# rlog58/dags-vae-search

Hardware: AMD Instinct MI355X
Metric: DAGs/sec VAE+predictor train step, n=12 batch 4096 per GPU, at 1 MI355X (higher is better)
Workload: dtype f32 (fwd bf16x6, bwd bf16x3 split products, fp32 accumulate); 1 GPU; synthetic_v12 DAGs (n=12, card=12, N=15 tokens), PACE-VAE train step: pack + fwd + bwd + clip_grad_norm_(1.0) + Adam(1e-4), train mode dropout 0.15; per_gpu_batch=4096, global_batch=4096, waves_per_workgroup=8, parallelism=single

## Files before the change

### dags_vae_search_amd/csrc/dvs_stage.h

```cpp
#pragma once
#include "dvs_device.h"

constexpr int DVS_PLAN_VECS = 6;
struct DvsStagePlan {
    const f4* src;
    int dst16;
    int n16;
    const float* vsrc[DVS_PLAN_VECS];
    unsigned short vdst[DVS_PLAN_VECS];
    unsigned short vbase[DVS_PLAN_VECS];
    unsigned short vlen[DVS_PLAN_VECS];
    int vperm;
    int nvec;
    int zero_int;
    int phase;
    const float* cold[2];
    int cold_tiles;
};

#ifdef DVS_STAMPS
constexpr int DVS_STAMP_IDS = 8, DVS_STAMP_PHASES = 32, DVS_STAMP_WAVES = 8, DVS_STAMP_WGS = 256;
#define DVS_STAMP_DECL(name) __device__ unsigned long long name[DVS_STAMP_WGS * DVS_STAMP_WAVES * DVS_STAMP_PHASES * DVS_STAMP_IDS]
#define DVS_STAMP(buf, pp, id)                                                                                              \
    do {                                                                                                                    \
        if ((dvs_tid() & 63) == 0 && dvs_bid() < DVS_STAMP_WGS && (dvs_tid() >> 6) < DVS_STAMP_WAVES)                        \
            buf[(((size_t)dvs_bid() * DVS_STAMP_WAVES + (dvs_tid() >> 6)) * DVS_STAMP_PHASES + ((pp)->phase & 31)) *          \
                    DVS_STAMP_IDS + (id)] = __builtin_amdgcn_s_memtime();                                                    \
    } while (0)
#define DVS_ACC_STAMP_DECL(name) __device__ unsigned long long name[256 * 8 * 8]
#define DVS_ACC_STAMP_AT(buf, last, nw, ids, k)                                                                             \
    do {                                                                                                                    \
        const unsigned long long now_ = __builtin_amdgcn_s_memtime();                                                       \
        if ((dvs_tid() & 63) == 0 && dvs_bid() < 256) buf[(dvs_bid() * (nw) + (dvs_tid() >> 6)) * (ids) + (k)] += now_ - last; \
        last = now_;                                                                                                        \
    } while (0)
#define DVS_ACC_STAMP(buf, last, k) DVS_ACC_STAMP_AT(buf, last, 8, 8, k)
#define DVS_STAMP_READER(name)                                                                                              \
    extern "C" int dvs_debug_read_stamps_##name(void* out, size_t bytes, int clear) {                                       \
        if (bytes > sizeof(dvs_stamps_##name)) bytes = sizeof(dvs_stamps_##name);                                           \
        if (hipMemcpyFromSymbol(out, HIP_SYMBOL(dvs_stamps_##name), bytes) != hipSuccess) return 1;                         \
        void* p = nullptr;                                                                                                  \
        if (clear && (hipGetSymbolAddress(&p, HIP_SYMBOL(dvs_stamps_##name)) != hipSuccess ||                               \
                      hipMemset(p, 0, sizeof(dvs_stamps_##name)) != hipSuccess))                                            \
            return 2;                                                                                                       \
        return 0;                                                                                                           \
    }
#else
#define DVS_STAMP(buf, pp, id) ((void)0)
#define DVS_ACC_STAMP(buf, last, k) ((void)0)
#define DVS_ACC_STAMP_AT(buf, last, nw, ids, k) ((void)0)
#endif

#ifndef DVS_EMU
#define DVS_HD __host__ __device__
#else
#define DVS_HD
#endif
#define DVS_FAKE_LDS ((char*)(uintptr_t)(1u << 20))
DVS_HD inline void dvs_plan_clear(DvsStagePlan& p) {
    p.src = nullptr;
    p.dst16 = 0;
    p.n16 = 0;
    for (int i = 0; i < DVS_PLAN_VECS; ++i) {
        p.vsrc[i] = nullptr;
        p.vdst[i] = 0;
        p.vbase[i] = 0;
        p.vlen[i] = 0;
    }
    p.phase = 0;
    p.nvec = 0;
    p.vperm = 0;
    p.zero_int = -1;
    p.cold[0] = p.cold[1] = nullptr;
    p.cold_tiles = 0;
}
DVS_HD inline void dvs_plan_cold(DvsStagePlan& p, const float* a, const float* b, int tiles) {
    p.cold[0] = a ? a : b;
    p.cold[1] = b ? b : a;
    p.cold_tiles = (a || b) ? tiles : 0;
}
DVS_HD inline void dvs_plan_seg(DvsStagePlan& p, const char* smem, const void* lds_dst, const void* src, int n_bf16) {
    p.src = (const f4*)src;
    p.dst16 = (int)(((const char*)lds_dst - smem) >> 4);
    p.n16 = n_bf16 >> 3;
}
DVS_HD inline void dvs_plan_vec(DvsStagePlan& p, const char* smem, const float* lds_dst, const float* src, int n,
                                bool perm = false) {
    for (int base = 0; base < n; base += 64) {
        if (p.nvec >= DVS_PLAN_VECS) {
            p.nvec = DVS_PLAN_VECS + 1;
            return;
        }
        p.vsrc[p.nvec] = src;
        p.vdst[p.nvec] = (unsigned short)(((const char*)lds_dst - smem) >> 2);
        p.vbase[p.nvec] = (unsigned short)base;
        p.vlen[p.nvec] = (unsigned short)n;
        if (perm) p.vperm |= 1 << p.nvec;
        ++p.nvec;
    }
}

constexpr int DVS_PF_THREADS = 256;
constexpr int DVS_PF_BWD = 9, DVS_PF_FWD = 14, DVS_PF_BWD_TAIL = 18, DVS_PF_FWD_TAIL = 27;
template <int NCH>
struct DvsPrefetch {
    f4 v[NCH];
    float s[2];
};

#ifndef DVS_EMU
typedef const __attribute__((address_space(4))) DvsStagePlan* DvsPlanK;
#else
typedef const DvsStagePlan* DvsPlanK;
#endif

DVS_HD inline bool dvs_plan_ok(const DvsStagePlan& p) { return p.nvec <= DVS_PLAN_VECS; }
void dvs_note_hip_error(const char* what, int hip_error, const char* hip_message);
DVS_HD inline void dvs_plan_seal(DvsStagePlan& p) {
#if !defined(__HIP_DEVICE_COMPILE__)
    if (!dvs_plan_ok(p)) {
        dvs_note_hip_error("staging plan", -1, "more than DVS_PLAN_VECS vector units (launcher bug)");
        p.nvec = DVS_PLAN_VECS;
    }
#endif
    for (int i = 0; i < DVS_PLAN_VECS; ++i)
        if (i >= p.nvec || !p.vsrc[i] || p.vlen[i] <= 0) {
            p.vsrc[i] = (const float*)p.src;
            p.vbase[i] = 0;
            p.vlen[i] = 0;
        }
}

__device__ __forceinline__ int dvs_uniform(int v) {
#ifndef DVS_EMU
    return __builtin_amdgcn_readfirstlane(v);
#else
    return v;
#endif
}
struct DvsPlanHead {
    const char* src;
    int dst, nwc, rot, wave, nw, lane16;
};
template <bool ROT, class PP>
__device__ __forceinline__ DvsPlanHead dvs_plan_head(PP p, int tid, int step) {
    DvsPlanHead h;
    h.src = (const char*)p->src;
    h.dst = p->dst16 * 16;
    h.nwc = p->n16 >> 6;
    h.rot = ROT ? (int)(((unsigned)dvs_bid() * 2654435761u) % (unsigned)(h.nwc > 0 ? h.nwc : 1)) : 0;
    h.wave = dvs_uniform(tid >> 6);
    h.nw = step >> 6;
    h.lane16 = (tid & 63) * 16;
    return h;
}
template <bool ROT>
__device__ __forceinline__ bool dvs_plan_slot(const DvsPlanHead& h, int u, int& byte) {
    int c = u * h.nw + h.wave;
    const bool live = c < h.nwc;
    if (ROT) {
        c += h.rot;
        c = c >= h.nwc ? c - h.nwc : c;
    }
    byte = ((live ? c : 0) << 10) + h.lane16;
    return live;
}

template <bool ROT, int NCH, class PP>
__device__ __forceinline__ void dvs_prefetch_issue(DvsPrefetch<NCH>& pf, PP p, int tid, int step) {
    const DvsPlanHead h = dvs_plan_head<ROT>(p, tid, step);
#pragma unroll
    for (int u = 0; u < NCH; ++u) {
        int byte;
        dvs_plan_slot<ROT>(h, u, byte);
        pf.v[u] = *(const f4*)(h.src + (unsigned)byte);
    }
#pragma unroll
    for (int q = 0; q < 2; ++q) {
        const int j = h.wave + q * h.nw, jc = j < DVS_PLAN_VECS ? j : 0;
        const int idx = p->vbase[jc] + (tid & 63);
        const int ic = (j < DVS_PLAN_VECS && idx < p->vlen[jc]) ? idx : 0;
        pf.s[q] = p->vsrc[jc][((p->vperm >> jc) & 1) ? dvs_pi(ic) : ic];
    }
}
template <bool ROT, int NCH, class PP>
__device__ __forceinline__ void dvs_prefetch_commit(const DvsPrefetch<NCH>& pf, PP p, char* smem, int tid, int step) {
    const DvsPlanHead h = dvs_plan_head<ROT>(p, tid, step);
#pragma unroll
    for (int u = 0; u < NCH; ++u) {
        int byte;
        if (dvs_plan_slot<ROT>(h, u, byte)) *(f4*)(smem + h.dst + byte) = pf.v[u];
    }
    float* ldsf = (float*)smem;
#pragma unroll
    for (int q = 0; q < 2; ++q) {
        const int j = h.wave + q * h.nw, jc = j < DVS_PLAN_VECS ? j : 0;
        const int idx = p->vbase[jc] + (tid & 63);
        if (j < DVS_PLAN_VECS && idx < p->vlen[jc]) ldsf[p->vdst[jc] + idx] = pf.s[q];
    }
    if (p->zero_int >= 0 && tid < 2) ((int*)smem)[p->zero_int + tid] = 0;
}
struct DvsTouch {
    float v[2];
};
template <class PP>
__device__ __forceinline__ DvsTouch dvs_touch_first(PP next, bool has_next, int nw, int wave, int lane) {
    DvsTouch t;
    t.v[0] = t.v[1] = 0.f;
    if (has_next && next->cold_tiles > 0) {
        int tile = dvs_bid() * nw + wave;
        tile = tile < next->cold_tiles ? tile : 0;
        const size_t off = (size_t)tile * 1024 + (size_t)lane * 16;
        t.v[0] = next->cold[0][off];
        t.v[1] = next->cold[1][off];
    }
    return t;
}
__device__ __forceinline__ void dvs_touch_done(const DvsTouch& t) {
#ifndef DVS_EMU
    asm volatile("" ::"v"(t.v[0]), "v"(t.v[1]));
#else
    (void)t;
#endif
}

template <int NCH, class PP>
__device__ __forceinline__ void dvs_stage_now(PP p, char* smem) {
    DvsPrefetch<NCH> pf;
    dvs_prefetch_issue<true>(pf, p, dvs_tid(), (int)blockDim.x);
    dvs_prefetch_commit<true>(pf, p, smem, dvs_tid(), (int)blockDim.x);
}
```

### dags_vae_search_amd/csrc/k_forward.hip

```cpp
#include "dvs_kernels.h"
#include "dvs_wimg.h"

constexpr int PACK_DAGS = 4;
__device__ __forceinline__ void pack_stream(float* dst, const float* __restrict__ src, size_t nfloats) {
    const size_t n4 = nfloats >> 2;
    size_t i = threadIdx.x;
    for (; i + 3 * blockDim.x < n4; i += 4 * blockDim.x) {
        f4 v[4];
#pragma unroll
        for (int u = 0; u < 4; ++u) v[u] = *(const f4*)(src + 4 * (i + u * blockDim.x));
#pragma unroll
        for (int u = 0; u < 4; ++u) *(f4*)(dst + 4 * (i + u * blockDim.x)) = v[u];
    }
    for (; i < n4; i += blockDim.x) *(f4*)(dst + 4 * i) = *(const f4*)(src + 4 * i);
    for (size_t i = 4 * n4 + threadIdx.x; i < nfloats; i += blockDim.x) dst[i] = src[i];
}
__global__ __launch_bounds__(8 * 16 * PACK_DAGS) void k_pack(PackArgs a) {
    DVS_DYN_LDS(smem);
    const int N = a.N, C = a.C;
    const int dag0 = blockIdx.x * PACK_DAGS;
    const int nd = (a.B - dag0 < PACK_DAGS) ? a.B - dag0 : PACK_DAGS;
    float* s_lab = (float*)smem;
    float* s_pos = s_lab + PACK_DAGS * 16 * 16;
    float* s_adj = s_pos + PACK_DAGS * 16 * 16;
    float* s_msk = s_adj + PACK_DAGS * 16 * 16;
    {
        const float* src[4] = {a.lab1h + (size_t)dag0 * N * C, a.pos1h + (size_t)dag0 * N * N, a.adj + (size_t)dag0 * N * N,
                               (const float*)(a.tmask + (size_t)dag0 * 8 * N * N)};
        float* dst[4] = {s_lab, s_pos, s_adj, s_msk};
        const int nf[4] = {nd * N * C, nd * N * N, nd * N * N, nd * 8 * N * N / 4};
        bool whole = true;
#pragma unroll
        for (int k = 0; k < 4; ++k) whole = whole && (nf[k] & 3) == 0 && (nf[k] >> 2) <= 2 * (int)blockDim.x;
        if (whole) {
            f4 v[4][2];
#pragma unroll
            for (int k = 0; k < 4; ++k)
#pragma unroll
                for (int u = 0; u < 2; ++u) {
                    const int i = (int)threadIdx.x + u * (int)blockDim.x;
                    v[k][u] = *(const f4*)(src[k] + 4 * (i < (nf[k] >> 2) ? i : 0));
                }
#pragma unroll
            for (int k = 0; k < 4; ++k)
#pragma unroll
                for (int u = 0; u < 2; ++u) {
                    const int i = (int)threadIdx.x + u * (int)blockDim.x;
                    if (i < (nf[k] >> 2)) *(f4*)(dst[k] + 4 * i) = v[k][u];
                }
        } else {
#pragma unroll
            for (int k = 0; k < 4; ++k) pack_stream(dst[k], src[k], (size_t)nf[k]);
        }
    }
    __syncthreads();
    const int h = threadIdx.x / (16 * PACK_DAGS), d = (threadIdx.x >> 4) % PACK_DAGS, i = threadIdx.x & 15;
    if (d >= nd) return;
    const uint8_t* msk = (const uint8_t*)s_msk;
    int bad = 0;
    if (h > 0) {
        if (i < N) {
            const uint8_t* m0 = msk + ((size_t)d * 8 * N + i) * N;
            const uint8_t* mh = msk + (((size_t)d * 8 + h) * N + i) * N;
            for (int j = 0; j < N; ++j)
                if ((mh[j] != 0) != (m0[j] != 0)) bad |= 2;
        }
        if (bad) atomicOr(a.status, bad);
        return;
    }
    int label = 0, pos = 0;
    unsigned parents = 0, allowed = 1u << i;
    if (i < N) {
        const float* lr = s_lab + ((size_t)d * N + i) * C;
        int ones = 0;
        for (int c = 0; c < C; ++c) {
            const float v = lr[c];
            if (v == 1.0f) { label = c; ++ones; } else if (v != 0.0f) bad |= 1;
        }
        if (ones != 1) bad |= 1;
        const float* pr = s_pos + ((size_t)d * N + i) * N;
        ones = 0;
        for (int c = 0; c < N; ++c) {
            const float v = pr[c];
            if (v == 1.0f) { pos = c; ++ones; } else if (v != 0.0f) bad |= 1;
        }
        if (ones != 1) bad |= 1;
        const float* ad = s_adj + (size_t)d * N * N;
        for (int j = 0; j < N; ++j)
            if (ad[j * N + i] != 0.0f) parents |= 1u << j;
        allowed = 0;
        const uint8_t* m0 = msk + ((size_t)d * 8 * N + i) * N;
        for (int j = 0; j < N; ++j)
            if (!m0[j]) allowed |= 1u << j;
        if (!((allowed >> i) & 1u)) bad |= 4;
    }
    DvsRecord* r = a.rec + dag0 + d;
    r->label[i] = (uint8_t)label;
    r->pos[i] = (uint8_t)pos;
    r->parents[i] = (uint16_t)parents;
    r->allowed[i] = (uint16_t)allowed;
    if (bad) atomicOr(a.status, bad);
}

void dvs_launch_pack(const PackArgs& a, dvs_stream_t st) {
    const size_t lds = (size_t)PACK_DAGS * (3 * 256 * 4 + 8 * 256);
    DVS_SET_LDS(k_pack, lds);
    DVS_LAUNCH(k_pack, dim3((a.B + PACK_DAGS - 1) / PACK_DAGS), dim3(8 * 16 * PACK_DAGS), lds, st, a);
}

__global__ __launch_bounds__(256) void k_build_records(BuildArgs a) {
    __shared__ unsigned short s_child[16][256];
    __shared__ unsigned short s_reach[16][256];
    __shared__ unsigned char s_indeg[16][256];
    __shared__ unsigned char s_order[16][256];
    const int tid = threadIdx.x;
    const int dag = blockIdx.x * 256 + tid;
    if (dag >= a.B) return;
    const int N = a.N, n = N - 3, out_id = N - 1;
    int bad = 0;
    for (int v = 0; v < 16; ++v) s_child[v][tid] = 0;
    s_child[0][tid] = 1u << 1;
    unsigned haspred = 0;
    for (int v = 0; v < n; ++v) {
        const unsigned p = a.preds[(size_t)dag * n + v];
        if (p >> v) bad |= 8;
        for (int u = 0; u < v; ++u)
            if ((p >> u) & 1u) s_child[u + 2][tid] |= (unsigned short)(1u << (v + 2));
        if (p & ((1u << v) - 1u)) haspred |= 1u << v;
    }
    for (int v = 0; v < n; ++v)
        if (!((haspred >> v) & 1u)) s_child[1][tid] |= (unsigned short)(1u << (v + 2));
    for (int v = 0; v < N - 1; ++v)
        if (s_child[v][tid] == 0) s_child[v][tid] = (unsigned short)(1u << out_id);
    for (int v = 0; v < 16; ++v) s_indeg[v][tid] = 0;
    for (int u = 0; u < N; ++u) {
        unsigned c = s_child[u][tid];
        while (c) {
            const int v = __ffs((int)c) - 1;
            c &= c - 1;
            s_indeg[v][tid]++;
        }
    }
    int tail = 0;
    for (int v = 0; v < N; ++v)
        if (s_indeg[v][tid] == 0) s_order[tail++][tid] = (unsigned char)v;
    for (int head = 0; head < tail && head < N; ++head) {
        unsigned c = s_child[s_order[head][tid]][tid];
        while (c) {
            const int v = __ffs((int)c) - 1;
            c &= c - 1;
            if (--s_indeg[v][tid] == 0 && tail < 16) s_order[tail++][tid] = (unsigned char)v;
        }
    }
    if (tail != N) bad |= 8;
    for (int v = 0; v < N; ++v) s_reach[v][tid] = (unsigned short)(s_child[v][tid] | (1u << v));
    for (int k = 0; k < N; ++k) {
        const unsigned rk = s_reach[k][tid];
        for (int v = 0; v < N; ++v)
            if ((s_reach[v][tid] >> k) & 1u) s_reach[v][tid] |= (unsigned short)rk;
    }
    DvsRecord* r = a.rec + dag;
    for (int i = 0; i < 16; ++i) {
        int label = 0, pos = 0;
        unsigned parents = 0, allowed = 1u << i;
        if (i < N) {
            if (i == 0) label = 2;
            else if (i == 1) label = 0;
            else if (i == out_id) label = 1;
            else {
                label = a.labels[(size_t)dag * n + (i - 2)] + 3;
                if (label >= a.C) { bad |= 1; label = 0; }
            }
            pos = s_order[i][tid];
            allowed = 0;
            for (int j = 0; j < N; ++j) {
                if ((s_child[j][tid] >> i) & 1u) parents |= 1u << j;
                if ((s_reach[j][tid] >> i) & 1u) allowed |= 1u << j;
            }
        }
        r->label[i] = (uint8_t)label;
        r->pos[i] = (uint8_t)pos;
        r->parents[i] = (uint16_t)parents;
        r->allowed[i] = (uint16_t)allowed;
    }
    if (bad) atomicOr(a.status, bad);
}

void dvs_launch_build_records(const BuildArgs& a, dvs_stream_t st) {
    DVS_LAUNCH(k_build_records, dim3((a.B + 255) / 256), dim3(256), 0, st, a);
}

struct EmbLds {
    float *W1, *W2, *labw, *labb, *scr;
};
__device__ __forceinline__ EmbLds emb_lds(char* smem) {
    EmbLds l;
    l.W1 = (float*)smem;
    l.W2 = l.W1 + 2 * DVS_MAXTOK * DVS_LD;
    l.labw = l.W2 + 64 * EMB_LDW2;
    l.labb = l.labw + 32 * 16;
    l.scr = l.labb + 32;
    return l;
}
static size_t emb_lds_floats(int nwaves) {
    const size_t n = 2 * DVS_MAXTOK * DVS_LD + 64 * EMB_LDW2 + 32 * 16 + 32 + (size_t)nwaves * 16;
    return n > (size_t)DvsEmbImg::FLOATS ? n : (size_t)DvsEmbImg::FLOATS;
}

__global__ __launch_bounds__(1024) void k_embed_fwd(EmbedArgs a, DvsStagePlan plan) {
    DVS_DYN_LDS(smem);
    const int N = a.dims.N, C = a.dims.C;
    const EmbLds l = emb_lds(smem);
    if (blockDim.x >= 1024) dvs_stage_now<2>(&plan, smem);
    else dvs_stage_now<5>(&plan, smem);
    __syncthreads();
    const Lane L = dvs_lane();
    const DvsDrop D = dvs_drop_of(a.dims);
    float* scr = l.scr + L.wave * 16;
    for (int dag = blockIdx.x * L.nwaves + L.wave; dag < a.dims.B; dag += gridDim.x * L.nwaves) {
        const DvsRecord* rec = a.rec + dag;
        const bool valid = L.r < N;
        const EmbSel sel = dvs_emb_selectors(rec, N, scr, L);
        f4 eh[4];
        dvs_emb_hidden(eh, l.W1, N, sel, L);
        const uint32_t gdag = a.dims.dag_offset + dag;
        const int label = rec->label[L.r];
        for (int v = 0; v < (a.out2 ? 2 : 1); ++v) {
            const int site = v ? a.site2 : a.site;
            f4 e1[4];
#pragma unroll
            for (int t = 0; t < 4; ++t) e1[t] = eh[t];
            dvs_dropout_tile(e1, dvs_site_key(a.dims.seed_lo, a.dims.seed_hi, site, gdag), D, L);
            f4 x[4];
            f4 e2[2] = {f4_zero(), f4_zero()};
#pragma unroll
            for (int t = 0; t < 4; ++t) {
                const f4 w0 = dvs_wcol(l.W2, EMB_LDW2, 0, t, L), w1 = dvs_wcol(l.W2, EMB_LDW2, 16, t, L);
#pragma unroll
                for (int kk = 0; kk < 4; ++kk) {
                    e2[0] = dvs_mfma(w0[kk], e1[t][kk], e2[0]);
                    e2[1] = dvs_mfma(w1[kk], e1[t][kk], e2[1]);
                }
            }
            {
                f4 tmp[2] = {e2[0], e2[1]};
                dvs_dropout_tile<2>(tmp, dvs_site_key(a.dims.seed_lo, a.dims.seed_hi, site + 1, gdag), D, L);
                x[2] = tmp[0];
                x[3] = tmp[1];
            }
#pragma unroll
            for (int t = 0; t < 2; ++t)
#pragma unroll
                for (int kk = 0; kk < 4; ++kk) {
                    const int f = 16 * t + 4 * L.g + kk;
                    x[t][kk] = valid ? fmaxf(l.labw[f * 16 + label] + l.labb[f], 0.f) : 0.f;
                }
            if (!valid) { x[2] = f4_zero(); x[3] = f4_zero(); }
            dvs_store_tile(v ? a.out2 : a.out, dag, x, L);
        }
    }
}

void dvs_launch_embed_fwd(const EmbedArgs& a, int grid, int nw, dvs_stream_t st) {
    const size_t lds = emb_lds_floats(16) * 4;
    DvsStagePlan plan;
    dvs_plan_clear(plan);
    dvs_plan_seg(plan, DVS_FAKE_LDS, DVS_FAKE_LDS, a.embimg, 2 * DvsEmbImg::FLOATS);
    dvs_plan_seal(plan);
    DVS_SET_LDS(k_embed_fwd, lds);
    DVS_LAUNCH(k_embed_fwd, dim3(grid), dim3(nw == 4 ? 256 : 1024), lds, st, a, plan);
}

#ifdef DVS_STAMPS
DVS_STAMP_DECL(dvs_stamps_fwd);
struct DvsLatTag { int phase; };
__device__ const DvsLatTag dvs_lat_tag = {6};
#define DVS_LAT_STAMP(id) DVS_STAMP(dvs_stamps_fwd, &dvs_lat_tag, id)
DVS_ACC_STAMP_DECL(dvs_stamps_attn);
#endif
#define ASTAMP(k) DVS_ACC_STAMP(dvs_stamps_attn, ast_, k)
#include "dvs_latent.h"
struct AttnLds {
    dvs_bf16 *Win, *Wout;
    float *inb, *outb, *lg, *lb;
};
DVS_HD inline AttnLds attn_lds(char* smem) {
    AttnLds l;
    l.Win = (dvs_bf16*)smem;
    l.Wout = l.Win + 3 * 192 * DVS_LDB;
    l.inb = (float*)(l.Wout + 3 * 64 * DVS_LDB);
    l.outb = l.inb + 192;
    l.lg = l.outb + 64;
    l.lb = l.lg + 64;
    return l;
}
static size_t attn_lds_bytes() { return 3 * 256 * DVS_LDB * sizeof(dvs_bf16) + (192 + 64 + 128) * sizeof(float); }

inline void attn_plan(DvsStagePlan& p, const AttnArgs& a, char* smem) {
    const AttnLds l = attn_lds(smem);
    dvs_plan_clear(p);
    dvs_plan_seg(p, smem, l.Win, (const dvs_bf16*)a.wimg + DvsAttnImg::Win, (int)(DvsAttnImg::WoutT - DvsAttnImg::Win));
    dvs_plan_vec(p, smem, l.inb, a.in_b, 192, true);
    dvs_plan_vec(p, smem, l.outb, a.out_b, 64);
    dvs_plan_vec(p, smem, l.lg, a.ln.g, a.ln.stats ? 64 : 0);
    dvs_plan_vec(p, smem, l.lb, a.ln.b, a.ln.stats ? 64 : 0);
    dvs_plan_seal(p);
}

__device__ __forceinline__ void attn_qkv(f4 (&q)[4], f4 (&k)[4], f4 (&v)[4], const Split3T& x, const Split3T& kv,
                                         const AttnLds& l, const Lane& L) {
#pragma unroll
    for (int t = 0; t < 4; ++t) {
        q[t] = dvs_vecT(l.inb, t, L);
        k[t] = dvs_vecT(l.inb + 64, t, L);
        v[t] = f4_splat(l.inb[128 + 16 * t + L.r]);
    }
    dvs_matb3<4>(q, x, l.Win, 192, 0, L);
    dvs_matb3<4>(k, kv, l.Win, 192, 64, L);
    dvs_matb3<4, true>(v, kv, l.Win, 192, 128, L);
    const float scale = 0.35355339059327373f;
#pragma unroll
    for (int t = 0; t < 4; ++t) q[t] *= scale;
}

__device__ __forceinline__ void attn_scores_T(f4 (&s)[8], const f4 (&q)[4], const f4 (&k)[4], const Lane& L) {
#pragma unroll
    for (int h = 0; h < 8; ++h) s[h] = f4_zero();
#pragma unroll
    for (int kk = 0; kk < 2; ++kk)
#pragma unroll
        for (int t = 0; t < 4; ++t) {
            s[2 * t] = dvs_mfma(k[t][kk], q[t][kk], s[2 * t]);
            s[2 * t + 1] = dvs_mfma(k[t][kk + 2], q[t][kk + 2], s[2 * t + 1]);
        }
}
__device__ __forceinline__ void attn_softmax_T(f4 (&p)[8], float (&m)[8], float (&den)[8], const f4 (&s)[8],
                                               unsigned allowed_r, const Lane& L) {
    bool ok[4];
#pragma unroll
    for (int reg = 0; reg < 4; ++reg) ok[reg] = (allowed_r >> (4 * L.g + reg)) & 1u;
#pragma unroll
    for (int h = 0; h < 8; ++h) {
        float mx = -3.0e38f;
#pragma unroll
        for (int reg = 0; reg < 4; ++reg) mx = ok[reg] ? fmaxf(mx, s[h][reg]) : mx;
        m[h] = mx;
    }
#pragma unroll
    for (int h = 0; h < 8; ++h) m[h] = dvs_max_x16(m[h]);
#pragma unroll
    for (int h = 0; h < 8; ++h) m[h] = dvs_max_x32(m[h]);
#pragma unroll
    for (int h = 0; h < 8; ++h) {
        float sum = 0.f;
#pragma unroll
        for (int reg = 0; reg < 4; ++reg) {
            p[h][reg] = ok[reg] ? __expf(s[h][reg] - m[h]) : 0.f;
            sum += p[h][reg];
        }
        den[h] = sum;
    }
#pragma unroll
    for (int h = 0; h < 8; ++h) den[h] = dvs_add_x16(den[h]);
#pragma unroll
    for (int h = 0; h < 8; ++h) den[h] = dvs_add_x32(den[h]);
#pragma unroll
    for (int h = 0; h < 8; ++h) p[h] *= (1.0f / den[h]);
}

__device__ __forceinline__ f4 attn_drop_T(f4 p, uint32_t key, int h, const DvsDrop& D, const Lane& L) {
    if (!D.on) return p;
    const uint32_t p0 = (uint32_t)((h * 16 + L.r) * 8 + 2 * L.g);
    const uint32_t h0 = dvs_draw(key, p0), h1 = dvs_draw(key, p0 + 1);
    p[0] = ((h0 & 0xFFFFu) >= D.thr16) ? p[0] * D.scale : 0.f;
    p[1] = ((h0 >> 16) >= D.thr16) ? p[1] * D.scale : 0.f;
    p[2] = ((h1 & 0xFFFFu) >= D.thr16) ? p[2] * D.scale : 0.f;
    p[3] = ((h1 >> 16) >= D.thr16) ? p[3] * D.scale : 0.f;
    return p;
}

template <class PP>
__device__ __forceinline__ void dvs_fwd_tail(PP next, bool has_next, char* smem, PP mine) {
    if (has_next) {
        DvsPrefetch<DVS_PF_FWD_TAIL> pf;
        const bool fetcher = dvs_tid() < DVS_PF_THREADS;
        if (fetcher) dvs_prefetch_issue<false>(pf, next, dvs_tid(), DVS_PF_THREADS);
        DVS_STAMP(dvs_stamps_fwd, mine, 3);
        dvs_lds_barrier();
        DVS_STAMP(dvs_stamps_fwd, mine, 4);
        if (fetcher) dvs_prefetch_commit<false>(pf, next, smem, dvs_tid(), DVS_PF_THREADS);
        DVS_STAMP(dvs_stamps_fwd, mine, 6);
    }
}

template <int NW, class PP>
__device__ __forceinline__ void dvs_attn_fwd_phase(const AttnArgs& a, char* smem, PP mine, bool stage_mine, PP next,
                                                   bool has_next) {
    const AttnLds l = attn_lds(smem);
    DVS_STAMP(dvs_stamps_fwd, mine, 0);
    if (stage_mine) {
        dvs_stage_now<(NW >= 8 ? DVS_PF_FWD : DVS_PF_FWD_TAIL)>(mine, smem);
        __syncthreads();
    }
    DVS_STAMP(dvs_stamps_fwd, mine, 1);
    const Lane L = dvs_lane();
    const DvsDrop D = dvs_drop_of(a.dims);
    const int N = a.dims.N;
#ifdef DVS_STAMPS
    unsigned long long ast_ = __builtin_amdgcn_s_memtime();
#endif
    bool gate = !stage_mine;
    for (int base = dvs_bid() * L.nwaves; base < a.dims.B; base += gridDim.x * L.nwaves) {
        const int dag = base + L.wave;
        if (dag >= a.dims.B) {
            DVS_PHASE_GATE(gate);
            continue;
        }
        ASTAMP(7);
        f4 x[4], dummy[4], kvt[4];
        float rstd;
        {
            DvsRawX rx;
            dvs_load_x_issue(rx, a.xin, a.ln, dag, L);
            if (a.kv) dvs_load_tile(kvt, a.kv, dag, L);
            DVS_PHASE_GATE(gate);
            dvs_load_x_finish<false>(x, dummy, rstd, rx, a.ln, l.lg, l.lb, N, L);
        }
#ifdef DVS_STAMPS
        asm volatile("s_waitcnt vmcnt(0)" ::: "memory");
#endif
        ASTAMP(0);
        f4 q[4], k[4], v[4];
        {
            const Split3T xs = dvs_split3_T(x);
            if (a.kv) {
                attn_qkv(q, k, v, xs, dvs_split3_T(kvt), l, L);
            } else {
                attn_qkv(q, k, v, xs, xs, l, L);
            }
        }
        ASTAMP(1);
        const unsigned allowed_r = a.rec[dag].allowed[L.r];
        const uint32_t gdag = a.dims.dag_offset + dag;
        const uint32_t kprob = dvs_site_key(a.dims.seed_lo, a.dims.seed_hi, a.site_prob, gdag);
        f4 s[8], p[8];
        float m[8], den[8];
        attn_scores_T(s, q, k, L);
        attn_softmax_T(p, m, den, s, allowed_r, L);
        ASTAMP(2);
#pragma unroll
        for (int h = 0; h < 8; ++h) p[h] = attn_drop_T(p[h], kprob, h, D, L);
        ASTAMP(3);
        f4 o[4];
        {
            f4 oa[4], ob[4];
#pragma unroll
            for (int t = 0; t < 4; ++t) oa[t] = ob[t] = f4_zero();
#pragma unroll
            for (int kk = 0; kk < 4; ++kk)
#pragma unroll
                for (int t = 0; t < 4; ++t) {
                    oa[t] = dvs_mfma(v[t][kk], p[2 * t][kk], oa[t]);
                    ob[t] = dvs_mfma(v[t][kk], p[2 * t + 1][kk], ob[t]);
                }
#pragma unroll
            for (int t = 0; t < 4; ++t) o[t] = f4{oa[t][0], oa[t][1], ob[t][2], ob[t][3]};
        }
        ASTAMP(4);
        f4 y[4];
#pragma unroll
        for (int t = 0; t < 4; ++t) y[t] = dvs_vecT(l.outb, t, L);
        dvs_matb3<4>(y, dvs_split3_T(o), l.Wout, 64, 0, L);
        ASTAMP(5);
        dvs_dropout_tile(y, dvs_site_key(a.dims.seed_lo, a.dims.seed_hi, a.site_post, gdag), D, L);
        const bool valid = L.r < N;
#pragma unroll
        for (int t = 0; t < 4; ++t)
#pragma unroll
            for (int kk = 0; kk < 4; ++kk) y[t][kk] = valid ? x[t][kk] + y[t][kk] : 0.f;
        dvs_store_pre(a.out_pre, a.out_stats, dag, y, L);
        ASTAMP(6);
    }
    DVS_PHASE_GATE(gate);
    DVS_STAMP(dvs_stamps_fwd, mine, 2);
    dvs_fwd_tail(next, has_next, smem, mine);
}

template <int NW>
__global__ __launch_bounds__(64 * NW) void k_attn_fwd(AttnArgs a, DvsStagePlan plan) {
    DVS_DYN_LDS(smem);
    dvs_attn_fwd_phase<NW>(a, smem, &plan, true, &plan, false);
}

void dvs_launch_attn_fwd(const AttnArgs& a, int grid, int nw, dvs_stream_t st) {
    const size_t lds = attn_lds_bytes();
    DvsStagePlan plan;
    attn_plan(plan, a, DVS_FAKE_LDS);
    if (nw == 4) {
        DVS_SET_LDS(k_attn_fwd<4>, lds);
        DVS_LAUNCH_AS("k_attn_fwd", k_attn_fwd<4>, dim3(grid), dim3(256), lds, st, a, plan);
    } else {
        DVS_SET_LDS(k_attn_fwd<8>, lds);
        DVS_LAUNCH_AS("k_attn_fwd", k_attn_fwd<8>, dim3(grid), dim3(512), lds, st, a, plan);
    }
}

struct FfnLds {
    dvs_bf16 *W1, *W2;
    float *b1, *b2, *lg, *lb, *ng, *nb;
};
DVS_HD inline FfnLds ffn_lds(char* smem) {
    FfnLds l;
    l.W1 = (dvs_bf16*)smem;
    l.W2 = l.W1 + 3 * 64 * DVS_LDB;
    l.b1 = (float*)(l.W2 + 3 * 64 * DVS_LDB);
    l.b2 = l.b1 + 64;
    l.lg = l.b2 + 64;
    l.lb = l.lg + 64;
    l.ng = l.lb + 64;
    l.nb = l.ng + 64;
    return l;
}
static size_t ffn_lds_bytes() { return 6 * 64 * DVS_LDB * sizeof(dvs_bf16) + 6 * 64 * sizeof(float); }

inline void ffn_plan(DvsStagePlan& p, const FfnArgs& a, char* smem) {
    const FfnLds l = ffn_lds(smem);
    dvs_plan_clear(p);
    dvs_plan_seg(p, smem, l.W1, (const dvs_bf16*)a.wimg + DvsFfnImg::W1, (int)(6 * DVS_IMG64));
    dvs_plan_vec(p, smem, l.b1, a.l1_b, 64);
    dvs_plan_vec(p, smem, l.b2, a.l2_b, 64);
    dvs_plan_vec(p, smem, l.lg, a.ln.g, a.ln.stats ? 64 : 0);
    dvs_plan_vec(p, smem, l.lb, a.ln.b, a.ln.stats ? 64 : 0);
    dvs_plan_vec(p, smem, l.ng, a.ng, a.out_norm ? 64 : 0);
    dvs_plan_vec(p, smem, l.nb, a.nb, a.out_norm ? 64 : 0);
    dvs_plan_seal(p);
}

template <class PP>
__device__ __forceinline__ void dvs_ffn_fwd_phase(const FfnArgs& a, char* smem, PP mine, bool stage_mine, PP next,
                                                  bool has_next) {
    const FfnLds l = ffn_lds(smem);
    DVS_STAMP(dvs_stamps_fwd, mine, 0);
    if (stage_mine) {
        dvs_stage_now<DVS_PF_FWD>(mine, smem);
        __syncthreads();
    }
    DVS_STAMP(dvs_stamps_fwd, mine, 1);
    const Lane L = dvs_lane();
    const DvsDrop D = dvs_drop_of(a.dims);
    const int ntiles = a.dims.B * a.dims.NT;
    bool gate = !stage_mine;
    for (int base = dvs_bid() * L.nwaves; base < ntiles; base += gridDim.x * L.nwaves) {
        const int tile = base + L.wave;
        if (tile >= ntiles) {
            DVS_PHASE_GATE(gate);
            continue;
        }
        const DvsTile T = dvs_tile_of(tile, a.dims);
        f4 x[4], dummy[4];
        float rstd;
        {
            DvsRawX rx;
            dvs_load_x_issue(rx, a.xin, a.ln, tile, L);
            DVS_PHASE_GATE(gate);
            dvs_load_x_finish<false>(x, dummy, rstd, rx, a.ln, l.lg, l.lb, T.Nl, L);
        }
        const uint32_t gdag = a.dims.dag_offset + T.dag;
        f4 h[4];
#pragma unroll
        for (int t = 0; t < 4; ++t) h[t] = dvs_vecT(l.b1, t, L);
        dvs_matb3<4>(h, dvs_split3_T(x), l.W1, 64, 0, L);
#pragma unroll
        for (int t = 0; t < 4; ++t)
#pragma unroll
            for (int kk = 0; kk < 4; ++kk) h[t][kk] = fmaxf(h[t][kk], 0.f);
        dvs_dropout_tile(h, dvs_site_key(a.dims.seed_lo, a.dims.seed_hi, a.site_hidden, gdag), D, L, T.tok0);
        f4 y[4];
#pragma unroll
        for (int t = 0; t < 4; ++t) y[t] = dvs_vecT(l.b2, t, L);
        dvs_matb3<4>(y, dvs_split3_T(h), l.W2, 64, 0, L);
        dvs_dropout_tile(y, dvs_site_key(a.dims.seed_lo, a.dims.seed_hi, a.site_post, gdag), D, L, T.tok0);
        const bool valid = L.r < T.Nl;
#pragma unroll
        for (int t = 0; t < 4; ++t)
#pragma unroll
            for (int kk = 0; kk < 4; ++kk) y[t][kk] = valid ? x[t][kk] + y[t][kk] : 0.f;
        float mean, rs;
        dvs_ln_stats(y, mean, rs);
        dvs_store_tile(a.out_pre, tile, y, L);
        if (L.g == 0) {
            a.out_stats[(size_t)tile * 32 + L.r] = mean;
            a.out_stats[(size_t)tile * 32 + 16 + L.r] = rs;
        }
        if (a.out_norm) {
            f4 xn[4];
#pragma unroll
            for (int t = 0; t < 4; ++t) {
                const f4 g = dvs_vecT(l.ng, t, L), b = dvs_vecT(l.nb, t, L);
#pragma unroll
                for (int kk = 0; kk < 4; ++kk) xn[t][kk] = valid ? (y[t][kk] - mean) * rs * g[kk] + b[kk] : 0.f;
            }
            dvs_store_tile(a.out_norm, tile, xn, L);
        }
    }
    DVS_PHASE_GATE(gate);
    DVS_STAMP(dvs_stamps_fwd, mine, 2);
    dvs_fwd_tail(next, has_next, smem, mine);
}

__global__ __launch_bounds__(1024) void k_ffn_fwd(FfnArgs a, DvsStagePlan plan) {
    DVS_DYN_LDS(smem);
    dvs_ffn_fwd_phase(a, smem, &plan, true, &plan, false);
}

void dvs_launch_ffn_fwd(const FfnArgs& a, int grid, int nw, dvs_stream_t st) {
    const size_t lds = ffn_lds_bytes();
    DvsStagePlan plan;
    ffn_plan(plan, a, DVS_FAKE_LDS);
    DVS_SET_LDS(k_ffn_fwd, lds);
    DVS_LAUNCH(k_ffn_fwd, dim3(grid), dim3(nw == 4 ? 256 : 1024), lds, st, a, plan);
}

template <int TAG, int NW>
__global__ __launch_bounds__(64 * NW) void k_fwd_stack(FwdStackArgs s) {
    DVS_DYN_LDS(smem);
#ifndef DVS_EMU
    const DvsPlanK plans =
        ((const __attribute__((address_space(4))) FwdStackArgs*)__builtin_amdgcn_kernarg_segment_ptr())->plan;
#else
    const DvsPlanK plans = s.plan;
#endif
    for (int i = 0; i < s.nphase; ++i) {
        const FwdPhase& ph = s.ph[i];
        const bool first = i == 0, more = i + 1 < s.nphase;
        const DvsPlanK mine = plans + i;
        if (TAG == 0 && NW == 8 && ph.kind == DVS_FPH_LATENT) {
            const int step = (int)gridDim.x * 8, B = ph.u.l.dims.B;
            for (int base = dvs_bid() * 8; base < B; base += 2 * step) {
                __syncthreads();
                dvs_latent_fwd_group(ph.u.l, smem, base, base + step);
            }
            continue;
        }
        const bool more_img = more && s.ph[i + 1].kind != DVS_FPH_LATENT;
        const DvsPlanK next = plans + (more_img ? i + 1 : i);
        if (ph.kind == DVS_FPH_ATTN) dvs_attn_fwd_phase<NW>(ph.u.a, smem, mine, first, next, more_img);
        else dvs_ffn_fwd_phase(ph.u.f, smem, mine, first, next, more_img);
    }
}

void dvs_launch_fwd_stack(const FwdStackArgs& s_in, int tag, int grid, int nw, dvs_stream_t st) {
    FwdStackArgs s = s_in;
    for (int i = 0; i < s.nphase; ++i) {
        if (s.ph[i].kind == DVS_FPH_ATTN) attn_plan(s.plan[i], s.ph[i].u.a, DVS_FAKE_LDS);
        else if (s.ph[i].kind == DVS_FPH_FFN) ffn_plan(s.plan[i], s.ph[i].u.f, DVS_FAKE_LDS);
        else dvs_plan_clear(s.plan[i]);
        s.plan[i].phase = i;
    }
#ifdef DVS_STAMPS
    for (int i = 0; i < s.nphase; ++i) s.plan[i].phase = tag * DVS_FWD_STACK_PHASES + i;
#endif
    const size_t la = attn_lds_bytes(), lf = ffn_lds_bytes();
    const size_t lds = la > lf ? la : lf;
#define DVS_FSTACK_LAUNCH(TG, NWV)                                                             \
    do {                                                                                       \
        DVS_SET_LDS((k_fwd_stack<TG, NWV>), lds);                                              \
        DVS_LAUNCH_AS("k_fwd_stack<" #TG ">", (k_fwd_stack<TG, NWV>), dim3(grid), dim3(64 * NWV), lds, st, s); \
    } while (0)
    if (nw == 4) {
        if (tag == 0) DVS_FSTACK_LAUNCH(0, 4);
        else DVS_FSTACK_LAUNCH(1, 4);
    } else {
        if (tag == 0) DVS_FSTACK_LAUNCH(0, 8);
        else DVS_FSTACK_LAUNCH(1, 8);
    }
}

__global__ void k_unfrag(const float* frag, float* out, int B) {
    const size_t i = (size_t)blockIdx.x * blockDim.x + threadIdx.x;
    if (i >= (size_t)B * 1024) return;
    const size_t dag = i >> 10;
    const int e = (int)(i & 1023);
    const int t = e >> 8, lane = (e >> 2) & 63, kk = e & 3;
    const int r = lane & 15, g = lane >> 4;
    out[dag * 1024 + r * 64 + 16 * t + 4 * g + kk] = frag[i];
}
void dvs_launch_unfrag(const float* frag, float* out, int B, dvs_stream_t st) {
    const size_t n = (size_t)B * 1024;
    DVS_LAUNCH(k_unfrag, dim3((unsigned)((n + 255) / 256)), dim3(256), 0, st, frag, out, B);
}

#ifdef DVS_STAMPS
DVS_STAMP_READER(attn)
DVS_STAMP_READER(fwd)
#endif
```

Baseline: 3.496 million DAGs/s.

## Ping-pong forward phase LDS regions and stage non-overlapping next-phase chunks early

Forward stack phases now alternate between the low and high ends of a fixed 160 KiB LDS allocation. The part of the next phase's staging that does not overlap the current phase's LDS region is loaded directly into LDS with global_load_lds, issued at the tail. Only the overlapping remainder goes through the register prefetch and commit after the barrier, which cuts register-held chunks and shortens the tail. In exchange, each workgroup uses much more LDS, which can lower occupancy. The plan also carries cut metadata that adds some per-phase address arithmetic.

After: 3.513 million DAGs/s (median of 6 runs). No clear change (+0.5%).

```diff
diff --git a/dags_vae_search_amd/csrc/dvs_stage.h b/dags_vae_search_amd/csrc/dvs_stage.h
--- a/dags_vae_search_amd/csrc/dvs_stage.h
+++ b/dags_vae_search_amd/csrc/dvs_stage.h
@@ -7,13 +7,20 @@
     int dst16;
     int n16;
     const float* vsrc[DVS_PLAN_VECS];
-    unsigned short vdst[DVS_PLAN_VECS];
-    unsigned short vbase[DVS_PLAN_VECS];
-    unsigned short vlen[DVS_PLAN_VECS];
+    union {
+        struct {
+            unsigned short vdst[DVS_PLAN_VECS];
+            unsigned short vbase[DVS_PLAN_VECS];
+            unsigned short vlen[DVS_PLAN_VECS];
+        };
+        unsigned vwords[3 * DVS_PLAN_VECS / 2];
+    };
     int vperm;
     int nvec;
     int zero_int;
     int phase;
+    int org16;
+    int early;
     const float* cold[2];
     int cold_tiles;
 };
@@ -68,6 +75,7 @@
         p.vlen[i] = 0;
     }
     p.phase = 0;
+    p.org16 = p.early = 0;
     p.nvec = 0;
     p.vperm = 0;
     p.zero_int = -1;
@@ -100,8 +108,32 @@
     }
 }
 
+DVS_HD inline void dvs_plan_shift(DvsStagePlan& p, int org) {
+    p.org16 = org >> 4;
+    p.dst16 += org >> 4;
+    for (int i = 0; i < DVS_PLAN_VECS; ++i) p.vdst[i] = (unsigned short)(p.vdst[i] + (org >> 2));
+    if (p.zero_int >= 0) p.zero_int += org >> 2;
+}
+struct DvsCut {
+    int e0, e1;
+};
+constexpr DvsCut dvs_cut(int dst, int nwc, int lo, int hi) {
+    int below = dst >= lo ? 0 : (lo - dst) >> 10;
+    int above = hi <= dst ? 0 : (hi - dst + 1023) >> 10;
+    below = below > nwc ? nwc : below;
+    above = above > nwc ? nwc : above;
+    return below >= nwc - above ? DvsCut{0, below} : DvsCut{above, nwc};
+}
+constexpr bool dvs_cut_ok(int dst, int nwc, int e0, int e1, int lo, int hi, int lds_bytes) {
+    if (e0 < 0 || e0 > e1 || e1 > nwc) return false;
+    if (e0 == e1) return true;
+    if (e0 != 0 && e1 != nwc) return false;
+    const int s = dst + (e0 << 10), t = dst + (e1 << 10);
+    return s >= 0 && t <= lds_bytes && (t <= lo || s >= hi);
+}
+
 constexpr int DVS_PF_THREADS = 256;
-constexpr int DVS_PF_BWD = 9, DVS_PF_FWD = 14, DVS_PF_BWD_TAIL = 18, DVS_PF_FWD_TAIL = 27;
+constexpr int DVS_PF_BWD = 9, DVS_PF_FWD = 14, DVS_PF_FWD_NARROW = 27, DVS_PF_BWD_TAIL = 18, DVS_PF_FWD_TAIL = 15;
 template <int NCH>
 struct DvsPrefetch {
     f4 v[NCH];
@@ -138,16 +170,23 @@
     return v;
 #endif
 }
+template <bool CUT, class PP>
+__device__ __forceinline__ int dvs_plan_v16(PP p, int k, int j) {
+    if (CUT) return (int)((p->vwords[k * (DVS_PLAN_VECS / 2) + (j >> 1)] >> ((j & 1) * 16)) & 0xFFFFu);
+    return k == 0 ? p->vdst[j] : k == 1 ? p->vbase[j] : p->vlen[j];
+}
 struct DvsPlanHead {
     const char* src;
-    int dst, nwc, rot, wave, nw, lane16;
-};
-template <bool ROT, class PP>
+    int dst, c0, nwc, rot, wave, nw, lane16;
+};
+template <bool ROT, bool CUT, class PP>
 __device__ __forceinline__ DvsPlanHead dvs_plan_head(PP p, int tid, int step) {
     DvsPlanHead h;
     h.src = (const char*)p->src;
     h.dst = p->dst16 * 16;
-    h.nwc = p->n16 >> 6;
+    const int all = p->n16 >> 6, cut = CUT ? p->early : 0, e0 = cut & 0xFFFF, e1 = cut >> 16;
+    h.nwc = e0 == 0 ? all - e1 : e0;
+    h.c0 = e0 == 0 && e1 < all ? e1 : 0;
     h.rot = ROT ? (int)(((unsigned)dvs_bid() * 2654435761u) % (unsigned)(h.nwc > 0 ? h.nwc : 1)) : 0;
     h.wave = dvs_uniform(tid >> 6);
     h.nw = step >> 6;
@@ -162,13 +201,13 @@
         c += h.rot;
         c = c >= h.nwc ? c - h.nwc : c;
     }
-    byte = ((live ? c : 0) << 10) + h.lane16;
+    byte = (((live ? c : 0) + h.c0) << 10) + h.lane16;
     return live;
 }
 
-template <bool ROT, int NCH, class PP>
+template <bool ROT, bool CUT = false, int NCH, class PP>
 __device__ __forceinline__ void dvs_prefetch_issue(DvsPrefetch<NCH>& pf, PP p, int tid, int step) {
-    const DvsPlanHead h = dvs_plan_head<ROT>(p, tid, step);
+    const DvsPlanHead h = dvs_plan_head<ROT, CUT>(p, tid, step);
 #pragma unroll
     for (int u = 0; u < NCH; ++u) {
         int byte;
@@ -178,14 +217,14 @@
 #pragma unroll
     for (int q = 0; q < 2; ++q) {
         const int j = h.wave + q * h.nw, jc = j < DVS_PLAN_VECS ? j : 0;
-        const int idx = p->vbase[jc] + (tid & 63);
-        const int ic = (j < DVS_PLAN_VECS && idx < p->vlen[jc]) ? idx : 0;
+        const int idx = dvs_plan_v16<CUT>(p, 1, jc) + (tid & 63);
+        const int ic = (j < DVS_PLAN_VECS && idx < dvs_plan_v16<CUT>(p, 2, jc)) ? idx : 0;
         pf.s[q] = p->vsrc[jc][((p->vperm >> jc) & 1) ? dvs_pi(ic) : ic];
     }
 }
-template <bool ROT, int NCH, class PP>
+template <bool ROT, bool CUT = false, int NCH, class PP>
 __device__ __forceinline__ void dvs_prefetch_commit(const DvsPrefetch<NCH>& pf, PP p, char* smem, int tid, int step) {
-    const DvsPlanHead h = dvs_plan_head<ROT>(p, tid, step);
+    const DvsPlanHead h = dvs_plan_head<ROT, CUT>(p, tid, step);
 #pragma unroll
     for (int u = 0; u < NCH; ++u) {
         int byte;
@@ -195,11 +234,33 @@
 #pragma unroll
     for (int q = 0; q < 2; ++q) {
         const int j = h.wave + q * h.nw, jc = j < DVS_PLAN_VECS ? j : 0;
-        const int idx = p->vbase[jc] + (tid & 63);
-        if (j < DVS_PLAN_VECS && idx < p->vlen[jc]) ldsf[p->vdst[jc] + idx] = pf.s[q];
+        const int idx = dvs_plan_v16<CUT>(p, 1, jc) + (tid & 63);
+        if (j < DVS_PLAN_VECS && idx < dvs_plan_v16<CUT>(p, 2, jc)) ldsf[dvs_plan_v16<CUT>(p, 0, jc) + idx] = pf.s[q];
     }
     if (p->zero_int >= 0 && tid < 2) ((int*)smem)[p->zero_int + tid] = 0;
 }
+template <class PP>
+__device__ __forceinline__ void dvs_early_issue(PP p, char* lds) {
+    const int tid = dvs_tid();
+    if (tid >= DVS_PF_THREADS) return;
+    const int cut = p->early, c1 = cut >> 16;
+    const char* src = (const char*)p->src + (tid & 63) * 16;
+    char* dst = lds + p->dst16 * 16;
+    for (int c = (cut & 0xFFFF) + dvs_uniform(tid >> 6); c < c1; c += DVS_PF_THREADS / 64) {
+#ifndef DVS_EMU
+        __builtin_amdgcn_global_load_lds((const __attribute__((address_space(1))) void*)(src + (c << 10)),
+                                         (__attribute__((address_space(3))) void*)(dst + (c << 10)), 16, 0, 0);
+#else
+        *(f4*)(dst + (c << 10) + (tid & 63) * 16) = *(const f4*)(src + (c << 10));
+#endif
+    }
+}
+__device__ __forceinline__ void dvs_early_retire() {
+#ifndef DVS_EMU
+    asm volatile("s_waitcnt vmcnt(0)" ::: "memory");
+#endif
+}
+
 struct DvsTouch {
     float v[2];
 };
diff --git a/dags_vae_search_amd/csrc/k_forward.hip b/dags_vae_search_amd/csrc/k_forward.hip
--- a/dags_vae_search_amd/csrc/k_forward.hip
+++ b/dags_vae_search_amd/csrc/k_forward.hip
@@ -294,7 +294,7 @@
     l.lb = l.lg + 64;
     return l;
 }
-static size_t attn_lds_bytes() { return 3 * 256 * DVS_LDB * sizeof(dvs_bf16) + (192 + 64 + 128) * sizeof(float); }
+constexpr size_t attn_lds_bytes() { return 3 * 256 * DVS_LDB * sizeof(dvs_bf16) + (192 + 64 + 128) * sizeof(float); }
 
 inline void attn_plan(DvsStagePlan& p, const AttnArgs& a, char* smem) {
     const AttnLds l = attn_lds(smem);
@@ -380,26 +380,33 @@
 }
 
 template <class PP>
-__device__ __forceinline__ void dvs_fwd_tail(PP next, bool has_next, char* smem, PP mine) {
+__device__ __forceinline__ void dvs_fwd_tail(PP next, bool has_next, char* lds, PP mine) {
     if (has_next) {
         DvsPrefetch<DVS_PF_FWD_TAIL> pf;
         const bool fetcher = dvs_tid() < DVS_PF_THREADS;
-        if (fetcher) dvs_prefetch_issue<false>(pf, next, dvs_tid(), DVS_PF_THREADS);
+        if (fetcher) {
+            dvs_early_issue(next, lds);
+            DVS_STAMP(dvs_stamps_fwd, mine, 7);
+            dvs_prefetch_issue<false, true>(pf, next, dvs_tid(), DVS_PF_THREADS);
+        }
         DVS_STAMP(dvs_stamps_fwd, mine, 3);
         dvs_lds_barrier();
         DVS_STAMP(dvs_stamps_fwd, mine, 4);
-        if (fetcher) dvs_prefetch_commit<false>(pf, next, smem, dvs_tid(), DVS_PF_THREADS);
+        if (fetcher) {
+            dvs_prefetch_commit<false, true>(pf, next, lds, dvs_tid(), DVS_PF_THREADS);
+            dvs_early_retire();
+        }
         DVS_STAMP(dvs_stamps_fwd, mine, 6);
     }
 }
 
 template <int NW, class PP>
-__device__ __forceinline__ void dvs_attn_fwd_phase(const AttnArgs& a, char* smem, PP mine, bool stage_mine, PP next,
+__device__ __forceinline__ void dvs_attn_fwd_phase(const AttnArgs& a, char* lds, PP mine, bool stage_mine, PP next,
                                                    bool has_next) {
-    const AttnLds l = attn_lds(smem);
+    const AttnLds l = attn_lds(lds + mine->org16 * 16);
     DVS_STAMP(dvs_stamps_fwd, mine, 0);
     if (stage_mine) {
-        dvs_stage_now<(NW >= 8 ? DVS_PF_FWD : DVS_PF_FWD_TAIL)>(mine, smem);
+        dvs_stage_now<(NW >= 8 ? DVS_PF_FWD : DVS_PF_FWD_NARROW)>(mine, lds);
         __syncthreads();
     }
     DVS_STAMP(dvs_stamps_fwd, mine, 1);
@@ -483,7 +490,7 @@
     }
     DVS_PHASE_GATE(gate);
     DVS_STAMP(dvs_stamps_fwd, mine, 2);
-    dvs_fwd_tail(next, has_next, smem, mine);
+    dvs_fwd_tail(next, has_next, lds, mine);
 }
 
 template <int NW>
@@ -521,7 +528,7 @@
     l.nb = l.ng + 64;
     return l;
 }
-static size_t ffn_lds_bytes() { return 6 * 64 * DVS_LDB * sizeof(dvs_bf16) + 6 * 64 * sizeof(float); }
+constexpr size_t ffn_lds_bytes() { return 6 * 64 * DVS_LDB * sizeof(dvs_bf16) + 6 * 64 * sizeof(float); }
 
 inline void ffn_plan(DvsStagePlan& p, const FfnArgs& a, char* smem) {
     const FfnLds l = ffn_lds(smem);
@@ -537,12 +544,12 @@
 }
 
 template <class PP>
-__device__ __forceinline__ void dvs_ffn_fwd_phase(const FfnArgs& a, char* smem, PP mine, bool stage_mine, PP next,
+__device__ __forceinline__ void dvs_ffn_fwd_phase(const FfnArgs& a, char* lds, PP mine, bool stage_mine, PP next,
                                                   bool has_next) {
-    const FfnLds l = ffn_lds(smem);
+    const FfnLds l = ffn_lds(lds + mine->org16 * 16);
     DVS_STAMP(dvs_stamps_fwd, mine, 0);
     if (stage_mine) {
-        dvs_stage_now<DVS_PF_FWD>(mine, smem);
+        dvs_stage_now<DVS_PF_FWD>(mine, lds);
         __syncthreads();
     }
     DVS_STAMP(dvs_stamps_fwd, mine, 1);
@@ -605,7 +612,7 @@
     }
     DVS_PHASE_GATE(gate);
     DVS_STAMP(dvs_stamps_fwd, mine, 2);
-    dvs_fwd_tail(next, has_next, smem, mine);
+    dvs_fwd_tail(next, has_next, lds, mine);
 }
 
 __global__ __launch_bounds__(1024) void k_ffn_fwd(FfnArgs a, DvsStagePlan plan) {
@@ -649,19 +656,50 @@
     }
 }
 
+constexpr int DVS_FWD_LDS = 160 * 1024;
+constexpr int dvs_fwd_bytes(int kind) { return (int)(kind == DVS_FPH_ATTN ? attn_lds_bytes() : ffn_lds_bytes()); }
+constexpr int dvs_fwd_chunks(int kind) { return kind == DVS_FPH_ATTN ? 3 * 256 * 144 / 1024 : 6 * 64 * 144 / 1024; }
+constexpr int dvs_fwd_org(int kind, int i) { return (i & 1) ? DVS_FWD_LDS - dvs_fwd_bytes(kind) : 0; }
+constexpr int dvs_fwd_late(int kc, int kn, int i) {
+    const int dst = dvs_fwd_org(kn, i + 1), n = dvs_fwd_chunks(kn), lo = dvs_fwd_org(kc, i), hi = lo + dvs_fwd_bytes(kc);
+    const DvsCut c = dvs_cut(dst, n, lo, hi);
+    return dvs_cut_ok(dst, n, c.e0, c.e1, lo, hi, DVS_FWD_LDS) ? n - (c.e1 - c.e0) : -1;
+}
+static_assert(dvs_fwd_late(DVS_FPH_ATTN, DVS_FPH_FFN, 0) == 5 && dvs_fwd_late(DVS_FPH_ATTN, DVS_FPH_FFN, 1) == 4, "attention -> FFN");
+static_assert(dvs_fwd_late(DVS_FPH_FFN, DVS_FPH_ATTN, 0) == 5 && dvs_fwd_late(DVS_FPH_FFN, DVS_FPH_ATTN, 1) == 4, "FFN -> attention");
+static_assert(dvs_fwd_late(DVS_FPH_ATTN, DVS_FPH_ATTN, 0) == 59 && dvs_fwd_late(DVS_FPH_ATTN, DVS_FPH_ATTN, 1) == 58, "self -> cross");
+static_assert(dvs_fwd_late(DVS_FPH_FFN, DVS_FPH_FFN, 0) == 0, "FFN -> FFN");
+static_assert(59 <= DVS_PF_FWD_TAIL * (DVS_PF_THREADS / 64), "the tail holds the largest late part");
+static_assert(!dvs_cut_ok(51712, 108, 58, 108, 0, 112128, DVS_FWD_LDS) && dvs_cut_ok(51712, 108, 59, 108, 0, 112128, DVS_FWD_LDS), "");
+static_assert(!dvs_cut_ok(0, 54, 0, 54, 51712, DVS_FWD_LDS, DVS_FWD_LDS) && !dvs_cut_ok(0, 108, 10, 20, 112128, DVS_FWD_LDS, DVS_FWD_LDS), "");
+static_assert(!dvs_cut_ok(107008, 54, 0, 56, 0, 56832, DVS_FWD_LDS), "past the end of the plan / of LDS");
+
 void dvs_launch_fwd_stack(const FwdStackArgs& s_in, int tag, int grid, int nw, dvs_stream_t st) {
     FwdStackArgs s = s_in;
     for (int i = 0; i < s.nphase; ++i) {
-        if (s.ph[i].kind == DVS_FPH_ATTN) attn_plan(s.plan[i], s.ph[i].u.a, DVS_FAKE_LDS);
-        else if (s.ph[i].kind == DVS_FPH_FFN) ffn_plan(s.plan[i], s.ph[i].u.f, DVS_FAKE_LDS);
+        const int kind = s.ph[i].kind;
+        if (kind == DVS_FPH_ATTN) attn_plan(s.plan[i], s.ph[i].u.a, DVS_FAKE_LDS);
+        else if (kind == DVS_FPH_FFN) ffn_plan(s.plan[i], s.ph[i].u.f, DVS_FAKE_LDS);
         else dvs_plan_clear(s.plan[i]);
         s.plan[i].phase = i;
+        if (kind == DVS_FPH_LATENT) continue;
+        DvsStagePlan& p = s.plan[i];
+        dvs_plan_shift(p, dvs_fwd_org(kind, i));
+        if (i == 0) continue;
+        const int lo = dvs_fwd_org(s.ph[i - 1].kind, i - 1), hi = lo + dvs_fwd_bytes(s.ph[i - 1].kind);
+        const DvsCut c = dvs_cut(p.dst16 * 16, p.n16 >> 6, lo, hi);
+        p.early = c.e0 | c.e1 << 16;
+        const int late = (p.n16 >> 6) - (c.e1 - c.e0);
+        if (!dvs_cut_ok(p.dst16 * 16, p.n16 >> 6, c.e0, c.e1, lo, hi, DVS_FWD_LDS) ||
+            late > DVS_PF_FWD_TAIL * (DVS_PF_THREADS / 64) || (p.n16 & 63) != 0) {
+            dvs_note_hip_error("staging plan", -1, "early / late cut of a forward phase does not fit (launcher bug)");
+            return;
+        }
     }
 #ifdef DVS_STAMPS
     for (int i = 0; i < s.nphase; ++i) s.plan[i].phase = tag * DVS_FWD_STACK_PHASES + i;
 #endif
-    const size_t la = attn_lds_bytes(), lf = ffn_lds_bytes();
-    const size_t lds = la > lf ? la : lf;
+    const size_t lds = DVS_FWD_LDS;
 #define DVS_FSTACK_LAUNCH(TG, NWV)                                                             \
     do {                                                                                       \
         DVS_SET_LDS((k_fwd_stack<TG, NWV>), lds);                                              \
```
